# svip-lab/impersonator

Hardware: NVIDIA H100
Metric: frames/sec @256x256 (per-frame inference hot path) (higher is better)
Workload: dtype f16 main product + e4m3 correction products (hi/lo split), f32 accumulate

## Files before the change

impersonator_b200/csrc/conv_tc.cu:

```cuda
#include <cuda.h>

#include <stdlib.h>

#include <algorithm>
#include <new>
#include <type_traits>

#include "common.cuh"

namespace {

constexpr int TILE_H = 16, TILE_W = 8;
constexpr int SWAP_N_TILE = 64;
constexpr int SWAP_TILE_H = 32;
constexpr int KCHUNK = 64;
constexpr int ROW_BYTES = TILE_W * 128;
constexpr int MAX_TAPS = 49;
constexpr int MAX_GROUP = 8;
constexpr int RING_BYTES = 200 * 1024;
constexpr int MAX_STAGES = 8;
constexpr int NUM_CONSUMERS = 256;
constexpr int NUM_THREADS = NUM_CONSUMERS + 128;
constexpr int MAX_N_TILE = 128;
static_assert(2 * 2 * (TILE_H + MAX_GROUP - 1) * ROW_BYTES + 2 * 2 * MAX_N_TILE * 128 <= RING_BYTES,
              "every plan needs two A and two B entries in the ring");
static_assert(2 * 2 * (SWAP_TILE_H + MAX_GROUP - 1) * ROW_BYTES + 2 * 2 * SWAP_N_TILE * 128 <= RING_BYTES,
              "every swapped plan needs two A and two B entries in the ring");
static_assert(SWAP_N_TILE * (SWAP_TILE_H * TILE_W) == MAX_N_TILE * (TILE_H * TILE_W), "same accumulator budget");

__host__ __device__ constexpr int tile_rows(int n_tile) { return n_tile == SWAP_N_TILE ? SWAP_TILE_H : TILE_H; }

struct ConvParams {
    CUtensorMap a_hi[4];
    CUtensorMap a_lo[4];
    CUtensorMap w_hi;
    CUtensorMap w_lo;
    int n_img, tiles_y, tiles_x, n_tiles_n;
    int dom_h, dom_w;
    int ntaps, chunks0, chunks1;
    signed char dy[MAX_TAPS], dx[MAX_TAPS], tmap[MAX_TAPS];
    short wtap[MAX_TAPS];
    int ngroups;
    signed char g_first[MAX_TAPS], g_cnt[MAX_TAPS];
    int a_rows;
    int a_stages, b_stages;
    float* out; int out_h, out_w, cout;
    int oy_mul, oy_add, ox_mul, ox_add;
    double* stats;
    float out_scale;
    int phase_cols;
};

template <int N_TILE, bool SPLIT>
struct Cfg {
    static constexpr int B_BYTES = N_TILE * 128;
    static constexpr int B_STAGE_BYTES = B_BYTES * (SPLIT ? 2 : 1);
    static constexpr int BAR_BYTES = 4 * MAX_STAGES * 8;
    static constexpr int STATS_PARTS = N_TILE < SWAP_N_TILE ? 8 : N_TILE == SWAP_N_TILE ? 2 : 0;
    static constexpr int STATS_BYTES = STATS_PARTS * N_TILE * 8;
    static constexpr int SMEM_BYTES = 1024 + RING_BYTES + BAR_BYTES + STATS_BYTES;
    static_assert(B_STAGE_BYTES % 1024 == 0, "B entries must keep the 1024-byte swizzle alignment");
    static_assert(SMEM_BYTES <= 227 * 1024, "exceeds the shared memory of a block");
};

__device__ __forceinline__ uint32_t smem_u32(const void* p) { return (uint32_t)__cvta_generic_to_shared(p); }

__device__ __forceinline__ void mbar_init(uint64_t* bar, uint32_t count) {
    asm volatile("mbarrier.init.shared::cta.b64 [%0], %1;" ::"r"(smem_u32(bar)), "r"(count));
}
__device__ __forceinline__ void mbar_expect_tx(uint64_t* bar, uint32_t bytes) {
    asm volatile("mbarrier.arrive.expect_tx.shared::cta.b64 _, [%0], %1;" ::"r"(smem_u32(bar)), "r"(bytes) : "memory");
}
__device__ __forceinline__ void mbar_arrive(uint64_t* bar) {
    asm volatile("mbarrier.arrive.shared::cta.b64 _, [%0];" ::"r"(smem_u32(bar)) : "memory");
}
__device__ __forceinline__ bool mbar_try_wait(uint64_t* bar, uint32_t parity) {
    uint32_t ok;
    asm volatile("{\n\t.reg .pred p;\n\t"
                 "mbarrier.try_wait.parity.shared::cta.b64 p, [%1], %2;\n\t"
                 "selp.u32 %0, 1, 0, p;\n\t}"
                 : "=r"(ok) : "r"(smem_u32(bar)), "r"(parity) : "memory");
    return ok != 0;
}
__device__ __forceinline__ void mbar_wait(uint64_t* bar, uint32_t parity) {
    if (mbar_try_wait(bar, parity)) return;
    const long long t0 = clock64();
    while (!mbar_try_wait(bar, parity)) {
        if (clock64() - t0 > 4000000000ll) __trap();
    }
}
__device__ __forceinline__ bool elect_one() {
    uint32_t pred;
    asm volatile("{\n\t.reg .pred P;\n\telect.sync _|P, 0xffffffff;\n\tselp.b32 %0, 1, 0, P;\n\t}" : "=r"(pred));
    return pred != 0;
}
__device__ __forceinline__ void fence_barrier_init() { asm volatile("fence.mbarrier_init.release.cluster;" ::: "memory"); }
__device__ __forceinline__ void fence_proxy_async() { asm volatile("fence.proxy.async.shared::cta;" ::: "memory"); }

__device__ __forceinline__ void tma_load_4d(const CUtensorMap* map, void* dst, uint64_t* bar, int c0, int c1, int c2, int c3) {
    asm volatile("cp.async.bulk.tensor.4d.shared::cluster.global.mbarrier::complete_tx::bytes [%0], [%1, {%3, %4, %5, %6}], [%2];"
                 :: "r"(smem_u32(dst)), "l"(map), "r"(smem_u32(bar)), "r"(c0), "r"(c1), "r"(c2), "r"(c3) : "memory");
}
__device__ __forceinline__ void tma_load_3d(const CUtensorMap* map, void* dst, uint64_t* bar, int c0, int c1, int c2) {
    asm volatile("cp.async.bulk.tensor.3d.shared::cluster.global.mbarrier::complete_tx::bytes [%0], [%1, {%3, %4, %5}], [%2];"
                 :: "r"(smem_u32(dst)), "l"(map), "r"(smem_u32(bar)), "r"(c0), "r"(c1), "r"(c2) : "memory");
}

__device__ __forceinline__ uint64_t make_desc(uint32_t smem_addr) {
    return (uint64_t)((smem_addr & 0x3FFFF) >> 4) | (1ull << 16) | (64ull << 32) | (1ull << 62);
}
__device__ __forceinline__ void wgmma_fence() { asm volatile("wgmma.fence.sync.aligned;" ::: "memory"); }
__device__ __forceinline__ void wgmma_commit() { asm volatile("wgmma.commit_group.sync.aligned;" ::: "memory"); }
template <int N>
__device__ __forceinline__ void wgmma_wait() { asm volatile("wgmma.wait_group.sync.aligned %0;" :: "n"(N) : "memory"); }
__device__ __forceinline__ void acc_fence(float& r) { asm volatile("" : "+f"(r) :: "memory"); }

template <int N> __device__ __forceinline__ void wgmma_f16(float* d, uint64_t da, uint64_t db);
template <int N> __device__ __forceinline__ void wgmma_e4m3(float* d, uint64_t da, uint64_t db);
template <> __device__ __forceinline__ void wgmma_f16<16>(float* d, uint64_t da, uint64_t db) {
    asm volatile("{\n\t.reg .pred p;\n\tsetp.ne.b32 p, %10, 0;\n\t"
                 "wgmma.mma_async.sync.aligned.m64n16k16.f32.f16.f16 {%0, %1, %2, %3, %4, %5, %6, %7}, %8, %9, p, 1, 1, 0, 0;\n\t}"
                 : "+f"(d[0]), "+f"(d[1]), "+f"(d[2]), "+f"(d[3]), "+f"(d[4]), "+f"(d[5]), "+f"(d[6]), "+f"(d[7])
                 : "l"(da), "l"(db), "r"(1));
}
template <> __device__ __forceinline__ void wgmma_f16<32>(float* d, uint64_t da, uint64_t db) {
    asm volatile("{\n\t.reg .pred p;\n\tsetp.ne.b32 p, %18, 0;\n\t"
                 "wgmma.mma_async.sync.aligned.m64n32k16.f32.f16.f16 {%0, %1, %2, %3, %4, %5, %6, %7, %8, %9, %10, %11, %12, %13, %14, %15}, %16, %17, p, 1, 1, 0, 0;\n\t}"
                 : "+f"(d[0]), "+f"(d[1]), "+f"(d[2]), "+f"(d[3]), "+f"(d[4]), "+f"(d[5]), "+f"(d[6]), "+f"(d[7]), "+f"(d[8]), "+f"(d[9]), "+f"(d[10]), "+f"(d[11]), "+f"(d[12]), "+f"(d[13]), "+f"(d[14]), "+f"(d[15])
                 : "l"(da), "l"(db), "r"(1));
}
template <> __device__ __forceinline__ void wgmma_f16<128>(float* d, uint64_t da, uint64_t db) {
    asm volatile("{\n\t.reg .pred p;\n\tsetp.ne.b32 p, %66, 0;\n\t"
                 "wgmma.mma_async.sync.aligned.m64n128k16.f32.f16.f16 {%0, %1, %2, %3, %4, %5, %6, %7, %8, %9, %10, %11, %12, %13, %14, %15, %16, %17, %18, %19, %20, %21, %22, %23, %24, %25, %26, %27, %28, %29, %30, %31, %32, %33, %34, %35, %36, %37, %38, %39, %40, %41, %42, %43, %44, %45, %46, %47, %48, %49, %50, %51, %52, %53, %54, %55, %56, %57, %58, %59, %60, %61, %62, %63}, %64, %65, p, 1, 1, 0, 0;\n\t}"
                 : "+f"(d[0]), "+f"(d[1]), "+f"(d[2]), "+f"(d[3]), "+f"(d[4]), "+f"(d[5]), "+f"(d[6]), "+f"(d[7]), "+f"(d[8]), "+f"(d[9]), "+f"(d[10]), "+f"(d[11]), "+f"(d[12]), "+f"(d[13]), "+f"(d[14]), "+f"(d[15]), "+f"(d[16]), "+f"(d[17]), "+f"(d[18]), "+f"(d[19]), "+f"(d[20]), "+f"(d[21]), "+f"(d[22]), "+f"(d[23]), "+f"(d[24]), "+f"(d[25]), "+f"(d[26]), "+f"(d[27]), "+f"(d[28]), "+f"(d[29]), "+f"(d[30]), "+f"(d[31]), "+f"(d[32]), "+f"(d[33]), "+f"(d[34]), "+f"(d[35]), "+f"(d[36]), "+f"(d[37]), "+f"(d[38]), "+f"(d[39]), "+f"(d[40]), "+f"(d[41]), "+f"(d[42]), "+f"(d[43]), "+f"(d[44]), "+f"(d[45]), "+f"(d[46]), "+f"(d[47]), "+f"(d[48]), "+f"(d[49]), "+f"(d[50]), "+f"(d[51]), "+f"(d[52]), "+f"(d[53]), "+f"(d[54]), "+f"(d[55]), "+f"(d[56]), "+f"(d[57]), "+f"(d[58]), "+f"(d[59]), "+f"(d[60]), "+f"(d[61]), "+f"(d[62]), "+f"(d[63])
                 : "l"(da), "l"(db), "r"(1));
}
template <> __device__ __forceinline__ void wgmma_e4m3<16>(float* d, uint64_t da, uint64_t db) {
    asm volatile("{\n\t.reg .pred p;\n\tsetp.ne.b32 p, %10, 0;\n\t"
                 "wgmma.mma_async.sync.aligned.m64n16k32.f32.e4m3.e4m3 {%0, %1, %2, %3, %4, %5, %6, %7}, %8, %9, p, 1, 1;\n\t}"
                 : "+f"(d[0]), "+f"(d[1]), "+f"(d[2]), "+f"(d[3]), "+f"(d[4]), "+f"(d[5]), "+f"(d[6]), "+f"(d[7])
                 : "l"(da), "l"(db), "r"(1));
}
template <> __device__ __forceinline__ void wgmma_e4m3<32>(float* d, uint64_t da, uint64_t db) {
    asm volatile("{\n\t.reg .pred p;\n\tsetp.ne.b32 p, %18, 0;\n\t"
                 "wgmma.mma_async.sync.aligned.m64n32k32.f32.e4m3.e4m3 {%0, %1, %2, %3, %4, %5, %6, %7, %8, %9, %10, %11, %12, %13, %14, %15}, %16, %17, p, 1, 1;\n\t}"
                 : "+f"(d[0]), "+f"(d[1]), "+f"(d[2]), "+f"(d[3]), "+f"(d[4]), "+f"(d[5]), "+f"(d[6]), "+f"(d[7]), "+f"(d[8]), "+f"(d[9]), "+f"(d[10]), "+f"(d[11]), "+f"(d[12]), "+f"(d[13]), "+f"(d[14]), "+f"(d[15])
                 : "l"(da), "l"(db), "r"(1));
}
template <> __device__ __forceinline__ void wgmma_e4m3<128>(float* d, uint64_t da, uint64_t db) {
    asm volatile("{\n\t.reg .pred p;\n\tsetp.ne.b32 p, %66, 0;\n\t"
                 "wgmma.mma_async.sync.aligned.m64n128k32.f32.e4m3.e4m3 {%0, %1, %2, %3, %4, %5, %6, %7, %8, %9, %10, %11, %12, %13, %14, %15, %16, %17, %18, %19, %20, %21, %22, %23, %24, %25, %26, %27, %28, %29, %30, %31, %32, %33, %34, %35, %36, %37, %38, %39, %40, %41, %42, %43, %44, %45, %46, %47, %48, %49, %50, %51, %52, %53, %54, %55, %56, %57, %58, %59, %60, %61, %62, %63}, %64, %65, p, 1, 1;\n\t}"
                 : "+f"(d[0]), "+f"(d[1]), "+f"(d[2]), "+f"(d[3]), "+f"(d[4]), "+f"(d[5]), "+f"(d[6]), "+f"(d[7]), "+f"(d[8]), "+f"(d[9]), "+f"(d[10]), "+f"(d[11]), "+f"(d[12]), "+f"(d[13]), "+f"(d[14]), "+f"(d[15]), "+f"(d[16]), "+f"(d[17]), "+f"(d[18]), "+f"(d[19]), "+f"(d[20]), "+f"(d[21]), "+f"(d[22]), "+f"(d[23]), "+f"(d[24]), "+f"(d[25]), "+f"(d[26]), "+f"(d[27]), "+f"(d[28]), "+f"(d[29]), "+f"(d[30]), "+f"(d[31]), "+f"(d[32]), "+f"(d[33]), "+f"(d[34]), "+f"(d[35]), "+f"(d[36]), "+f"(d[37]), "+f"(d[38]), "+f"(d[39]), "+f"(d[40]), "+f"(d[41]), "+f"(d[42]), "+f"(d[43]), "+f"(d[44]), "+f"(d[45]), "+f"(d[46]), "+f"(d[47]), "+f"(d[48]), "+f"(d[49]), "+f"(d[50]), "+f"(d[51]), "+f"(d[52]), "+f"(d[53]), "+f"(d[54]), "+f"(d[55]), "+f"(d[56]), "+f"(d[57]), "+f"(d[58]), "+f"(d[59]), "+f"(d[60]), "+f"(d[61]), "+f"(d[62]), "+f"(d[63])
                 : "l"(da), "l"(db), "r"(1));
}

__device__ __forceinline__ void consumer_sync() { asm volatile("bar.sync 1, 256;" ::: "memory"); }

struct TileCoord {
    int n_idx, img, y0, x0;
};
template <int TH>
__device__ __forceinline__ TileCoord decode_tile(const ConvParams& P, int tile, int m_tiles) {
    TileCoord t;
    t.n_idx = tile / m_tiles;
    const int m_idx = tile % m_tiles;
    t.img = m_idx / (P.tiles_y * P.tiles_x);
    const int rem = m_idx % (P.tiles_y * P.tiles_x);
    t.y0 = (rem / P.tiles_x) * TH; t.x0 = (rem % P.tiles_x) * TILE_W;
    return t;
}

template <int N_TILE>
__device__ __forceinline__ void warp_tile_stats(const float* acc, bool v0, bool v1, int warp, unsigned lane, float2* s_stats)
{
#pragma unroll
    for (int j = 0; j < N_TILE / 8; j++) {
        const float a0 = v0 ? acc[4 * j] : 0.f, a1 = v0 ? acc[4 * j + 1] : 0.f;
        const float b0 = v1 ? acc[4 * j + 2] : 0.f, b1 = v1 ? acc[4 * j + 3] : 0.f;
        float s0 = a0 + b0, s1 = a1 + b1, q0 = a0 * a0 + b0 * b0, q1 = a1 * a1 + b1 * b1;
#pragma unroll
        for (int off = 4; off <= 16; off <<= 1) {
            s0 += __shfl_xor_sync(0xffffffffu, s0, off); s1 += __shfl_xor_sync(0xffffffffu, s1, off);
            q0 += __shfl_xor_sync(0xffffffffu, q0, off); q1 += __shfl_xor_sync(0xffffffffu, q1, off);
        }
        if (lane < 4) {
            s_stats[warp * N_TILE + 8 * j + 2 * lane] = make_float2(s0, q0);
            s_stats[warp * N_TILE + 8 * j + 2 * lane + 1] = make_float2(s1, q1);
        }
    }
}

template <int N_TILE, int PARTS>
__device__ __forceinline__ void flush_tile_stats(const ConvParams& P, const float2* s_stats, int img, int n_idx)
{
    consumer_sync();
    for (int col = threadIdx.x; col < N_TILE; col += NUM_CONSUMERS) {
        float s = 0.f, q = 0.f;
#pragma unroll
        for (int w = 0; w < PARTS; w++) { const float2 v = s_stats[w * N_TILE + col]; s += v.x; q += v.y; }
        int ch = n_idx * N_TILE + col;
        if (P.phase_cols > 0) ch %= P.phase_cols;
        double* dst = P.stats + 2 * ((size_t)img * P.cout + ch);
        atomicAdd(dst, (double)s);
        atomicAdd(dst + 1, (double)q);
    }
    consumer_sync();
}

template <int N_TILE>
__device__ __forceinline__ void epilogue_plain(const ConvParams& P, float* acc, const TileCoord& t, int warp, unsigned lane,
                                               float2* s_stats)
{
    const int tx = (int)(lane >> 2), x = t.x0 + tx;
    const int y[2] = {t.y0 + 2 * warp, t.y0 + 2 * warp + 1};
    const bool valid[2] = {y[0] < P.dom_h && x < P.dom_w, y[1] < P.dom_h && x < P.dom_w};
    if (P.out_scale != 1.f) {
#pragma unroll
        for (int i = 0; i < N_TILE / 2; i++) acc[i] *= P.out_scale;
    }
    if (P.out) {
        const int out_w_c = P.out_w * P.cout;
#pragma unroll
        for (int h = 0; h < 2; h++) {
            if (!valid[h]) continue;
            float* optr = P.out + (((size_t)t.img * P.out_h + (P.oy_mul * y[h] + P.oy_add)) * P.out_w + (P.ox_mul * x + P.ox_add)) * P.cout
                        + (size_t)t.n_idx * N_TILE;
#pragma unroll
            for (int j = 0; j < N_TILE / 8; j++) {
                const int c = 8 * j + 2 * (int)(lane & 3);
                float* o = optr + c;
                if (P.phase_cols > 0) {
                    const int col = t.n_idx * N_TILE + c, ph = col / P.phase_cols;
                    o = P.out + (((size_t)t.img * P.out_h + 2 * y[h]) * P.out_w + 2 * x) * P.cout
                      + (size_t)(ph >> 1) * out_w_c + (ph & 1) * P.cout + (col - ph * P.phase_cols);
                }
                *reinterpret_cast<float2*>(o) = make_float2(acc[4 * j + 2 * h], acc[4 * j + 2 * h + 1]);
            }
        }
    }
    if (P.stats) {
        warp_tile_stats<N_TILE>(acc, valid[0], valid[1], warp, lane, s_stats);
        flush_tile_stats<N_TILE, 8>(P, s_stats, t.img, t.n_idx);
    }
}

template <int N_TILE>
__device__ __forceinline__ void epilogue_channel_major(const ConvParams& P, float* acc, const TileCoord& t, int warp,
                                                       unsigned lane, float2* s_stats)
{
    const int wg = warp >> 2;
    const int c_base = N_TILE == MAX_N_TILE ? 64 * wg : 0, row0 = N_TILE == MAX_N_TILE ? 0 : 16 * wg;
    const int c0 = c_base + 16 * (warp & 3) + (int)(lane >> 2);
    const int y0 = t.y0 + row0, x0 = t.x0 + 2 * (int)(lane & 3);
    const int rows = P.dom_h - y0;
    const bool vx[2] = {x0 < P.dom_w, x0 + 1 < P.dom_w};
    const int col = t.n_idx * N_TILE + c0;
    const int ph = P.phase_cols > 0 ? col / P.phase_cols : 0;
    const int ch = col - ph * P.phase_cols;
    const size_t coff = ((size_t)(ph >> 1) * P.out_w + (ph & 1)) * P.cout + ch;
    if (P.out_scale != 1.f) {
#pragma unroll
        for (int i = 0; i < 64; i++) acc[i] *= P.out_scale;
    }
    if (P.out) {
#pragma unroll
        for (int j = 0; j < 16; j++) {
            if (j >= rows) break;
            const size_t orow = ((size_t)t.img * P.out_h + (P.oy_mul * (y0 + j) + P.oy_add)) * P.out_w;
#pragma unroll
            for (int e = 0; e < 2; e++) {
                if (!vx[e]) continue;
                float* o = P.out + (orow + (P.ox_mul * (x0 + e) + P.ox_add)) * P.cout;
                o[coff] = acc[4 * j + e];
                o[coff + 8] = acc[4 * j + 2 + e];
            }
        }
    }
    if (P.stats) {
        float s[2] = {0.f, 0.f}, q[2] = {0.f, 0.f};
#pragma unroll
        for (int j = 0; j < 16; j++) {
#pragma unroll
            for (int e = 0; e < 2; e++) {
                const bool v = j < rows && vx[e];
#pragma unroll
                for (int h = 0; h < 2; h++) {
                    const float a = v ? acc[4 * j + 2 * h + e] : 0.f;
                    s[h] += a; q[h] += a * a;
                }
            }
        }
#pragma unroll
        for (int h = 0; h < 2; h++) {
#pragma unroll
            for (int off = 1; off <= 2; off <<= 1) {
                s[h] += __shfl_xor_sync(0xffffffffu, s[h], off);
                q[h] += __shfl_xor_sync(0xffffffffu, q[h], off);
            }
        }
        if constexpr (N_TILE == SWAP_N_TILE) {
            if ((lane & 3) == 0) {
                s_stats[wg * N_TILE + c0] = make_float2(s[0], q[0]);
                s_stats[wg * N_TILE + c0 + 8] = make_float2(s[1], q[1]);
            }
            flush_tile_stats<N_TILE, 2>(P, s_stats, t.img, t.n_idx);
        } else if ((lane & 3) == 0) {
#pragma unroll
            for (int h = 0; h < 2; h++) {
                double* dst = P.stats + 2 * ((size_t)t.img * P.cout + ch + 8 * h);
                atomicAdd(dst, (double)s[h]);
                atomicAdd(dst + 1, (double)q[h]);
            }
        }
    }
}

enum { MODE_FP16 = 0, MODE_FP16X3 = 1, MODE_F8 = 2 };

template <int N_TILE, int MODE>
struct Regs {
    static constexpr int CONSUMER = N_TILE >= 64 ? (MODE == MODE_F8 ? 168 : 120) : N_TILE == 32 ? 80 : 64;
    static constexpr int LAUNCH = ((2 * CONSUMER + 40 + 2) / 3 + 7) / 8 * 8;
    static constexpr int PRODUCER = 3 * LAUNCH - 2 * CONSUMER;
    static_assert(PRODUCER >= 40 && PRODUCER % 8 == 0 && CONSUMER % 8 == 0, "setmaxnreg takes multiples of 8");
};

template <int N_TILE, bool CM>
__device__ __forceinline__ void mma_f16(float* d, uint64_t act, uint64_t w) {
    if constexpr (CM) wgmma_f16<128>(d, w, act);
    else              wgmma_f16<N_TILE>(d, act, w);
}
template <int N_TILE, bool CM>
__device__ __forceinline__ void mma_e4m3(float* d, uint64_t act, uint64_t w) {
    if constexpr (CM) wgmma_e4m3<128>(d, w, act);
    else              wgmma_e4m3<N_TILE>(d, act, w);
}

template <int N_TILE, int MODE>
__global__ void __launch_bounds__(NUM_THREADS, 1) __maxnreg__((Regs<N_TILE, MODE>::LAUNCH))
k_conv_wg(const __grid_constant__ ConvParams P)
{
    constexpr bool CM = N_TILE >= SWAP_N_TILE;
    constexpr bool SPLIT = MODE != MODE_FP16;
    constexpr int TH = N_TILE == SWAP_N_TILE ? SWAP_TILE_H : TILE_H;
    constexpr int ACC = CM ? 64 : N_TILE / 2;
    using C = Cfg<N_TILE, SPLIT>;
    extern __shared__ uint8_t smem_raw[];
    uint8_t* smem = reinterpret_cast<uint8_t*>((reinterpret_cast<uintptr_t>(smem_raw) + 1023) & ~(uintptr_t)1023);
    const int a_op_bytes = P.a_rows * ROW_BYTES;
    const int a_stage_bytes = a_op_bytes * (SPLIT ? 2 : 1);
    uint8_t* b_ring = smem + P.a_stages * a_stage_bytes;
    uint64_t* a_full = reinterpret_cast<uint64_t*>(smem + RING_BYTES);
    uint64_t* a_empty = a_full + MAX_STAGES;
    uint64_t* b_full = a_empty + MAX_STAGES;
    uint64_t* b_empty = b_full + MAX_STAGES;
    float2* s_stats = reinterpret_cast<float2*>(smem + RING_BYTES + C::BAR_BYTES);

    const int warp = threadIdx.x >> 5;
    const unsigned lane = threadIdx.x & 31;

    if (threadIdx.x == 0) {
        for (int s = 0; s < P.a_stages; s++) { mbar_init(a_full + s, 1); mbar_init(a_empty + s, NUM_CONSUMERS / 32); }
        for (int s = 0; s < P.b_stages; s++) { mbar_init(b_full + s, 1); mbar_init(b_empty + s, NUM_CONSUMERS / 32); }
        fence_barrier_init();
        fence_proxy_async();
    }
    __syncthreads();
    lwb::pdl_wait();
    lwb::pdl_trigger();

    const int nchunks = P.chunks0 + P.chunks1;
    const int m_tiles = P.n_img * P.tiles_y * P.tiles_x;
    const int total = m_tiles * P.n_tiles_n;

    if (warp >= NUM_CONSUMERS / 32) {
        asm volatile("setmaxnreg.dec.sync.aligned.u32 %0;" :: "n"(Regs<N_TILE, MODE>::PRODUCER));
        if (warp != NUM_CONSUMERS / 32) return;
        if (elect_one()) {
            asm volatile("prefetch.tensormap [%0];" :: "l"(&P.a_hi[0]) : "memory");
            asm volatile("prefetch.tensormap [%0];" :: "l"(&P.w_hi) : "memory");
            if (SPLIT) {
                asm volatile("prefetch.tensormap [%0];" :: "l"(&P.a_lo[0]) : "memory");
                asm volatile("prefetch.tensormap [%0];" :: "l"(&P.w_lo) : "memory");
            }
        }
        int as = 0, bs = 0; uint32_t aph = 0, bph = 0;
        for (int tile = blockIdx.x; tile < total; tile += gridDim.x) {
            const TileCoord t = decode_tile<TH>(P, tile, m_tiles);
            for (int g = 0; g < P.ngroups; g++) {
                const int first = P.g_first[g], cnt = P.g_cnt[g];
                const int xx = t.x0 + P.dx[first], yy = t.y0 + P.dy[first];
                for (int chunk = 0; chunk < nchunks; chunk++) {
                    const bool second = chunk >= P.chunks0;
                    const int mi = second ? 1 : P.tmap[first];
                    const int c0 = (second ? chunk - P.chunks0 : chunk) * KCHUNK;
                    mbar_wait(a_empty + as, aph ^ 1);
                    uint8_t* sa = smem + as * a_stage_bytes;
                    if (elect_one()) {
                        mbar_expect_tx(a_full + as, (uint32_t)a_stage_bytes);
                        tma_load_4d(&P.a_hi[mi], sa, a_full + as, c0, xx, yy, t.img);
                        if (SPLIT) tma_load_4d(&P.a_lo[mi], sa + a_op_bytes, a_full + as, c0, xx, yy, t.img);
                    }
                    __syncwarp();
                    if (++as == P.a_stages) { as = 0; aph ^= 1; }
                    for (int i = 0; i < cnt; i++) {
                        mbar_wait(b_empty + bs, bph ^ 1);
                        uint8_t* sb = b_ring + bs * C::B_STAGE_BYTES;
                        const int wt = P.wtap[first + i];
                        if (elect_one()) {
                            mbar_expect_tx(b_full + bs, (uint32_t)C::B_STAGE_BYTES);
                            tma_load_3d(&P.w_hi, sb, b_full + bs, chunk * KCHUNK, t.n_idx * N_TILE, wt);
                            if (SPLIT) tma_load_3d(&P.w_lo, sb + C::B_BYTES, b_full + bs, chunk * KCHUNK, t.n_idx * N_TILE, wt);
                        }
                        __syncwarp();
                        if (++bs == P.b_stages) { bs = 0; bph ^= 1; }
                    }
                }
            }
        }
    } else {
        asm volatile("setmaxnreg.inc.sync.aligned.u32 %0;" :: "n"(Regs<N_TILE, MODE>::CONSUMER));
        constexpr bool CH_SPLIT = N_TILE == MAX_N_TILE;
        const uint32_t wg = (uint32_t)(warp >> 2);
        const uint32_t a_base = smem_u32(smem) + (CH_SPLIT ? 0 : wg * (TH / 2) * ROW_BYTES);
        const uint32_t b_base = smem_u32(b_ring) + (CH_SPLIT ? wg * 64 * 128 : 0);
        float acc[ACC];
        float acc8[MODE == MODE_F8 ? ACC : 1];
        int as = 0, bs = 0; uint32_t aph = 0, bph = 0;
        for (int tile = blockIdx.x; tile < total; tile += gridDim.x) {
            const TileCoord t = decode_tile<TH>(P, tile, m_tiles);
#pragma unroll
            for (int i = 0; i < ACC; i++) acc[i] = 0.f;
#pragma unroll
            for (int i = 0; i < (MODE == MODE_F8 ? ACC : 1); i++) acc8[i] = 0.f;
            int prev_b = -1, prev_a = -1;
            for (int g = 0; g < P.ngroups; g++) {
                const int cnt = P.g_cnt[g];
                for (int chunk = 0; chunk < nchunks; chunk++) {
                    mbar_wait(a_full + as, aph);
                    const uint32_t a_hi = a_base + as * a_stage_bytes;
                    for (int i = 0; i < cnt; i++) {
                        mbar_wait(b_full + bs, bph);
                        const uint32_t ai = a_hi + i * ROW_BYTES, al = ai + a_op_bytes;
                        const uint32_t b_hi = b_base + bs * C::B_STAGE_BYTES, b_lo = b_hi + C::B_BYTES;
                        wgmma_fence();
#pragma unroll
                        for (int k = 0; k < KCHUNK / 16; k++) {
                            const uint64_t da = make_desc(ai + k * 32), db = make_desc(b_hi + k * 32);
                            mma_f16<N_TILE, CM>(acc, da, db);
                            if constexpr (MODE == MODE_F8) {
                                mma_e4m3<N_TILE, CM>(acc8, make_desc(al + k * 32), make_desc(b_lo + k * 32));
                            } else if constexpr (MODE == MODE_FP16X3) {
                                mma_f16<N_TILE, CM>(acc, da, make_desc(b_lo + k * 32));
                                mma_f16<N_TILE, CM>(acc, make_desc(al + k * 32), db);
                            }
                        }
                        wgmma_commit();
                        if (prev_b >= 0) {
                            wgmma_wait<1>();
                            if (lane == 0) {
                                mbar_arrive(b_empty + prev_b);
                                if (prev_a >= 0) mbar_arrive(a_empty + prev_a);
                            }
                            prev_a = -1;
                        }
                        prev_b = bs;
                        if (++bs == P.b_stages) { bs = 0; bph ^= 1; }
                    }
                    prev_a = as;
                    if (++as == P.a_stages) { as = 0; aph ^= 1; }
                }
            }
            wgmma_wait<0>();
#pragma unroll
            for (int i = 0; i < ACC; i++) acc_fence(acc[i]);
            if constexpr (MODE == MODE_F8) {
#pragma unroll
                for (int i = 0; i < ACC; i++) { acc_fence(acc8[i]); acc[i] += acc8[i]; }
            }
            if (lane == 0) { mbar_arrive(b_empty + prev_b); mbar_arrive(a_empty + prev_a); }
            if constexpr (CM) epilogue_channel_major<N_TILE>(P, acc, t, warp, lane, s_stats);
            else              epilogue_plain<N_TILE>(P, acc, t, warp, lane, s_stats);
        }
    }
}

typedef CUresult (*EncodeTiledFn)(CUtensorMap*, CUtensorMapDataType, cuuint32_t, void*, const cuuint64_t*,
                                  const cuuint64_t*, const cuuint32_t*, const cuuint32_t*, CUtensorMapInterleave,
                                  CUtensorMapSwizzle, CUtensorMapL2promotion, CUtensorMapFloatOOBfill);

EncodeTiledFn get_encode()
{
    static EncodeTiledFn fn = nullptr;
    if (!fn) {
        void* p = nullptr;
        cudaDriverEntryPointQueryResult q;
        if (cudaGetDriverEntryPoint("cuTensorMapEncodeTiled", &p, cudaEnableDefault, &q) != cudaSuccess || !p) return nullptr;
        fn = (EncodeTiledFn)p;
    }
    return fn;
}

int encode_map(CUtensorMap* m, const void* base, int rank, const uint64_t* dims, const uint64_t* strides_bytes, const uint32_t* box)
{
    EncodeTiledFn enc = get_encode();
    if (!enc) { lwb::set_error("cuTensorMapEncodeTiled entry point not available"); return LWB_E_CUDA; }
    cuuint64_t gdim[5]; cuuint64_t gstr[4]; cuuint32_t bx[5]; cuuint32_t es[5];
    for (int i = 0; i < rank; i++) { gdim[i] = dims[i]; bx[i] = box[i]; es[i] = 1; }
    for (int i = 0; i < rank - 1; i++) gstr[i] = strides_bytes[i];
    CUresult r = enc(m, CU_TENSOR_MAP_DATA_TYPE_FLOAT16, (cuuint32_t)rank, const_cast<void*>(base), gdim, gstr, bx, es,
                     CU_TENSOR_MAP_INTERLEAVE_NONE, CU_TENSOR_MAP_SWIZZLE_128B, CU_TENSOR_MAP_L2_PROMOTION_L2_256B,
                     CU_TENSOR_MAP_FLOAT_OOB_FILL_NONE);
    if (r != CUDA_SUCCESS) {
        lwb::set_error("cuTensorMapEncodeTiled failed (%d): rank %d dims [%llu,%llu,%llu,%llu] strides [%llu,%llu,%llu] box [%u,%u,%u,%u]",
                       (int)r, rank, (unsigned long long)dims[0], (unsigned long long)dims[1], (unsigned long long)(rank > 2 ? dims[2] : 0),
                       (unsigned long long)(rank > 3 ? dims[3] : 0), (unsigned long long)strides_bytes[0],
                       (unsigned long long)(rank > 2 ? strides_bytes[1] : 0), (unsigned long long)(rank > 3 ? strides_bytes[2] : 0),
                       box[0], box[1], rank > 2 ? box[2] : 0, rank > 3 ? box[3] : 0);
        return LWB_E_CUDA;
    }
    return LWB_OK;
}

struct Launch {
    ConvParams p;
    int n_tile;
    int mode;
    int grid;
};

template <int N_TILE, int MODE>
int launch_wg(const Launch& L, cudaStream_t st)
{
    using C = Cfg<N_TILE, MODE != MODE_FP16>;
    static bool attr_set_dev[lwb::kMaxDevices] = {};
    bool& attr_set = attr_set_dev[lwb::device_slot()];
    if (!attr_set) {
        LWB_CUDA_OK(cudaFuncSetAttribute(k_conv_wg<N_TILE, MODE>, cudaFuncAttributeMaxDynamicSharedMemorySize, C::SMEM_BYTES));
        attr_set = true;
    }
    LWB_CUDA_OK(lwb::launch_pdl(k_conv_wg<N_TILE, MODE>, dim3(L.grid), dim3(NUM_THREADS), C::SMEM_BYTES, st, L.p));
    LWB_LAUNCH_OK();
    return LWB_OK;
}

template <class F>
int with_instance(int n_tile, int mode, F&& f)
{
    auto modes = [&](auto nt) {
        if (mode == MODE_F8) return f(nt, std::integral_constant<int, MODE_F8>());
        if (mode == MODE_FP16X3) return f(nt, std::integral_constant<int, MODE_FP16X3>());
        return f(nt, std::integral_constant<int, MODE_FP16>());
    };
    switch (n_tile) {
        case 16:  return modes(std::integral_constant<int, 16>());
        case 32:  return modes(std::integral_constant<int, 32>());
        case 64:  return modes(std::integral_constant<int, 64>());
        case 128: return modes(std::integral_constant<int, 128>());
    }
    lwb::set_error("conv_tc: unsupported N tile %d", n_tile);
    return LWB_E_UNSUPPORTED;
}

int launch(const Launch& L, cudaStream_t st)
{
    return with_instance(L.n_tile, L.mode,
                         [&](auto nt, auto md) { return launch_wg<decltype(nt)::value, decltype(md)::value>(L, st); });
}

int pick_n_tile(int cout, int forced)
{
    if (forced > 0) return forced > MAX_N_TILE && forced % MAX_N_TILE == 0 ? MAX_N_TILE : forced;
    if (cout % 128 == 0) return 128;
    if (cout % 64 == 0) return 64;
    if (cout % 32 == 0) return 32;
    if (cout % 16 == 0) return 16;
    return -1;
}

struct View {
    const uint16_t* hi;
    const uint16_t* lo;
    uint64_t dims[4], str[3];
};

struct LaunchSpec {
    int ntaps;
    signed char dy[MAX_TAPS], dx[MAX_TAPS], tmap[MAX_TAPS];
    short wtap[MAX_TAPS];
    int chunks0, chunks1;
    int nviews;
    View a[4];
    View w;
    int ncols;
    int dom_h, dom_w;
    int oy_mul, oy_add, ox_mul, ox_add, phase_cols;
    int n_tile;

    void tap(int y, int x, int view, int wt)
    {
        dy[ntaps] = (signed char)y; dx[ntaps] = (signed char)x; tmap[ntaps] = (signed char)view; wtap[ntaps] = (short)wt;
        ntaps++;
    }
};

}

struct lwb_conv_plan {
    int num;
    Launch launches[4];
};

static View nhwc_view(const uint16_t* hi, const uint16_t* lo, int n, int h, int w, int c, int step = 1, int py = 0, int px = 0)
{
    const size_t off = ((size_t)py * w + px) * c;
    return View{hi + off, lo ? lo + off : lo,
                {(uint64_t)c, (uint64_t)((w - px + step - 1) / step), (uint64_t)((h - py + step - 1) / step), (uint64_t)n},
                {(uint64_t)step * c * 2, (uint64_t)step * w * c * 2, (uint64_t)h * w * c * 2}};
}

static View weight_view(const uint16_t* hi, const uint16_t* lo, int k, int ncols, int taps)
{
    return View{hi, lo, {(uint64_t)k, (uint64_t)ncols, (uint64_t)taps}, {(uint64_t)k * 2, (uint64_t)ncols * k * 2}};
}

static int encode_pair(CUtensorMap* hi, CUtensorMap* lo, int rank, const View& v, const uint32_t* box, bool split)
{
    const int rc = encode_map(hi, v.hi, rank, v.dims, v.str, box);
    return rc != LWB_OK || !split ? rc : encode_map(lo, v.lo, rank, v.dims, v.str, box);
}

static void group_taps(ConvParams& p, int tile_h)
{
    int order[MAX_TAPS];
    for (int t = 0; t < p.ntaps; t++) order[t] = t;
    std::stable_sort(order, order + p.ntaps, [&](int a, int b) {
        if (p.tmap[a] != p.tmap[b]) return p.tmap[a] < p.tmap[b];
        if (p.dx[a] != p.dx[b]) return p.dx[a] < p.dx[b];
        return p.dy[a] < p.dy[b];
    });
    const ConvParams src = p;
    int longest = 0;
    p.ngroups = 0;
    for (int t = 0; t < p.ntaps; t++) {
        const int o = order[t];
        p.dy[t] = src.dy[o]; p.dx[t] = src.dx[o]; p.tmap[t] = src.tmap[o]; p.wtap[t] = src.wtap[o];
        const bool joins = t > 0 && p.tmap[t] == p.tmap[t - 1] && p.dx[t] == p.dx[t - 1] && p.dy[t] == p.dy[t - 1] + 1 &&
                           p.g_cnt[p.ngroups - 1] < MAX_GROUP;
        if (!joins) { p.g_first[p.ngroups] = (signed char)t; p.g_cnt[p.ngroups] = 0; p.ngroups++; }
        p.g_cnt[p.ngroups - 1]++;
        longest = std::max(longest, (int)p.g_cnt[p.ngroups - 1]);
    }
    p.a_rows = tile_h + longest - 1;
}

static void pick_rings(ConvParams& p, int n_tile, bool split)
{
    const int ops = split ? 2 : 1;
    const int a_bytes = p.a_rows * ROW_BYTES * ops, b_bytes = n_tile * 128 * ops;
    const int longest = p.a_rows - tile_rows(n_tile) + 1;
    int best = 0;
    for (int a = 2; a <= MAX_STAGES; a++) {
        const int b = std::min(MAX_STAGES, (RING_BYTES - a * a_bytes) / b_bytes);
        if (b < 2) break;
        if (std::min(a * longest, b) > best) { best = std::min(a * longest, b); p.a_stages = a; p.b_stages = b; }
    }
}

static int build_launch(Launch& L, const LaunchSpec& s, const lwb_conv_desc* d, float* out_raw, double* stats, int sms)
{
    const bool split = d->split != 0;
    ConvParams& p = L.p;
    memset(&p, 0, sizeof(p));
    p.ntaps = s.ntaps; p.chunks0 = s.chunks0; p.chunks1 = s.chunks1;
    for (int t = 0; t < s.ntaps; t++) { p.dy[t] = s.dy[t]; p.dx[t] = s.dx[t]; p.tmap[t] = s.tmap[t]; p.wtap[t] = s.wtap[t]; }
    group_taps(p, tile_rows(s.n_tile));
    int rc;
    const uint32_t a_box[4] = {KCHUNK, TILE_W, (uint32_t)p.a_rows, 1};
    for (int v = 0; v < s.nviews; v++)
        if ((rc = encode_pair(&p.a_hi[v], &p.a_lo[v], 4, s.a[v], a_box, split)) != LWB_OK) return rc;
    const uint32_t w_box[3] = {KCHUNK, (uint32_t)s.n_tile, 1};
    if ((rc = encode_pair(&p.w_hi, &p.w_lo, 3, s.w, w_box, split)) != LWB_OK) return rc;
    p.n_img = d->n;
    p.dom_h = s.dom_h; p.dom_w = s.dom_w;
    p.tiles_y = lwb::ceil_div(s.dom_h, tile_rows(s.n_tile)); p.tiles_x = lwb::ceil_div(s.dom_w, TILE_W);
    p.n_tiles_n = s.ncols / s.n_tile;
    p.out = out_raw; p.out_h = d->h_out; p.out_w = d->w_out; p.cout = d->cout;
    p.oy_mul = s.oy_mul; p.oy_add = s.oy_add; p.ox_mul = s.ox_mul; p.ox_add = s.ox_add; p.phase_cols = s.phase_cols;
    p.stats = stats;
    p.out_scale = ldexpf(1.f, -d->w_exp);
    L.n_tile = s.n_tile; L.mode = d->split;
    pick_rings(p, s.n_tile, split);
    const long total = (long)p.n_img * p.tiles_y * p.tiles_x * p.n_tiles_n;
    L.grid = (int)(total < sms ? total : sms);
    return LWB_OK;
}

extern "C" int lwb_conv_plan_create(const lwb_conv_desc* d,
                                    const uint16_t* x0_hi, const uint16_t* x0_lo,
                                    const uint16_t* x1_hi, const uint16_t* x1_lo,
                                    const uint16_t* w_hi, const uint16_t* w_lo,
                                    float* out_raw, double* stats, lwb_conv_plan** plan_out)
{
    LWB_CHECK_ARG(d && x0_hi && w_hi && out_raw && plan_out, "null pointer");
    const bool split = d->split != 0;
    const bool f8 = d->split == 2;
    LWB_CHECK_ARG(d->split >= 0 && d->split <= 2, "split must be 0, 1 or 2");
    LWB_CHECK_ARG(!split || (x0_lo && w_lo), "split mode needs the lo operands");
    LWB_CHECK_ARG(!f8 || (!d->rowk && !d->halo), "the fp8 lo mode is not available for row-K / halo plans");
    LWB_CHECK_ARG(d->n > 0 && d->h_in > 0 && d->w_in > 0 && d->cout > 0, "non-positive size");
    LWB_CHECK_ARG(d->cout % 16 == 0, "cout must be a multiple of 16");
    LWB_CHECK_ARG(d->w_exp >= -40 && d->w_exp <= 60, "w_exp out of range");
    const int n_tile = pick_n_tile(d->cout, d->n_tile);
    LWB_CHECK_ARG(n_tile > 0 && d->cout % n_tile == 0, "no N tile divides cout");
    if (d->halo) {
        LWB_CHECK_ARG(d->stride == 1 && !d->transposed && d->dil == 1, "halo mode needs stride 1, dilation 1, not transposed");
        if (d->rowk) LWB_CHECK_ARG(d->kw <= 8 && d->cin0 == 8 && d->cin1 == 0 && d->row_pitch >= d->w_in + 8, "row-K shape");
        else         LWB_CHECK_ARG(d->kw <= 9 && (d->kw & 1) && (d->kh & 1), "halo mode needs an odd kernel, kw <= 9, with 'same' padding (kh/2, kw/2)");
    }

    const int sms = lwb::sm_count();

    LaunchSpec s = {};
    s.n_tile = n_tile; s.ncols = d->cout;
    s.dom_h = d->h_out; s.dom_w = d->w_out;
    s.oy_mul = s.ox_mul = 1;
    s.nviews = 1;
    LaunchSpec specs[4];
    int num = 1;
    if (d->rowk) {
        LWB_CHECK_ARG(d->stride == 1 && !d->transposed && d->kw <= 8 && d->cin0 == 8 && d->cin1 == 0, "row-K needs stride 1, kw <= 8, 8 channels");
        LWB_CHECK_ARG(d->h_out == d->h_in && d->w_out == d->w_in && d->row_pitch >= d->w_in + 8, "row-K shape");
        for (int ky = 0; ky < d->kh; ky++) s.tap(ky, 0, 0, ky);
        s.chunks0 = 1;
        const uint64_t hp = d->h_in + d->kh - 1, row_bytes = (uint64_t)d->row_pitch * 16;
        s.a[0] = View{x0_hi, x0_lo, {64, (uint64_t)d->w_in, hp, (uint64_t)d->n}, {16, row_bytes, hp * row_bytes}};
        s.w = weight_view(w_hi, w_lo, 64, d->cout, d->kh);
    } else {
        LWB_CHECK_ARG(d->cin0 % KCHUNK == 0 && d->cin1 % KCHUNK == 0 && d->cin0 > 0, "input channels must be multiples of 64");
        LWB_CHECK_ARG(d->cin1 == 0 || (x1_hi && (!split || x1_lo)), "second input missing");
        const int cin_total = d->cin0 + d->cin1;
        const int ntaps_w = d->kh * d->kw;
        LWB_CHECK_ARG(ntaps_w <= MAX_TAPS, "too many filter taps");
        s.chunks0 = d->cin0 / KCHUNK; s.chunks1 = d->cin1 / KCHUNK;
        s.a[0] = nhwc_view(x0_hi, x0_lo, d->n, d->h_in, d->w_in, d->cin0);
        s.w = weight_view(w_hi, w_lo, cin_total, d->cout, ntaps_w);
        if (d->transposed) {
            LWB_CHECK_ARG(d->kh == 3 && d->kw == 3 && d->stride == 2 && d->pad == 1 && d->cin1 == 0, "transposed conv: only k3 s2 p1 op1");
            LWB_CHECK_ARG(d->h_out == 2 * d->h_in && d->w_out == 2 * d->w_in, "transposed conv output must be 2x input");
            s.dom_h = d->h_in; s.dom_w = d->w_in;
            s.oy_mul = s.ox_mul = 2;
        }
        if (d->transposed == 2) {
            s.n_tile = MAX_N_TILE;
            s.ncols = 4 * d->cout;
            LWB_CHECK_ARG(d->cout % 32 == 0 && s.ncols % s.n_tile == 0, "merged transposed conv needs cout in multiples of 32");
            for (int t = 0; t < 4; t++) s.tap(t >> 1, t & 1, 0, t);
            s.w = weight_view(w_hi, w_lo, cin_total, s.ncols, 4);
            s.phase_cols = d->cout;
        } else if (d->transposed) {
            const int ky_list[2][2] = {{1, -1}, {2, 0}}, d_list[2][2] = {{0, 0}, {0, 1}}, cnt[2] = {1, 2};
            num = 4;
            for (int a = 0; a < 2; a++) for (int b = 0; b < 2; b++) {
                LaunchSpec& q = specs[a * 2 + b];
                q = s;
                for (int i = 0; i < cnt[a]; i++) for (int j = 0; j < cnt[b]; j++)
                    q.tap(d_list[a][i], d_list[b][j], 0, ky_list[a][i] * 3 + ky_list[b][j]);
                q.oy_add = a; q.ox_add = b;
            }
        } else {
            LWB_CHECK_ARG(d->stride == 1 || d->stride == 2, "stride must be 1 or 2");
            LWB_CHECK_ARG(d->stride == 1 || d->cin1 == 0, "concat input only with stride 1");
            const int st = d->stride;
            for (int ky = 0; ky < d->kh; ky++) for (int kx = 0; kx < d->kw; kx++) {
                const int oy = ky * d->dil - d->pad, ox = kx * d->dil - (d->pad_w >= 0 ? d->pad_w : d->pad);
                if (oy < -127 || oy > 127 || ox < -127 || ox > 127) { lwb::set_error("conv_tc: tap offset out of range"); return LWB_E_UNSUPPORTED; }
                const int py = ((oy % st) + st) % st, px = ((ox % st) + st) % st;
                s.tap((oy - py) / st, (ox - px) / st, py * 2 + px, s.ntaps);
            }
            s.nviews = st * st;
            for (int v = 0; v < s.nviews; v++) s.a[v] = nhwc_view(x0_hi, x0_lo, d->n, d->h_in, d->w_in, d->cin0, st, v >> 1, v & 1);
            if (d->cin1) {
                s.nviews = 2;
                s.a[1] = nhwc_view(x1_hi, x1_lo, d->n, d->h_in, d->w_in, d->cin1);
            }
        }
    }
    if (num == 1) specs[0] = s;

    lwb_conv_plan* plan = new (std::nothrow) lwb_conv_plan();
    LWB_CHECK_ARG(plan, "out of host memory");
    for (; plan->num < num; plan->num++) {
        const int rc = build_launch(plan->launches[plan->num], specs[plan->num], d, out_raw, stats, sms);
        if (rc != LWB_OK) { delete plan; return rc; }
    }
    *plan_out = plan;
    return LWB_OK;
}

extern "C" int lwb_conv_plan_run(const lwb_conv_plan* plan, lwb_stream_t stream)
{
    LWB_CHECK_ARG(plan, "null plan");
    for (int i = 0; i < plan->num; i++) {
        const int rc = launch(plan->launches[i], (cudaStream_t)stream);
        if (rc != LWB_OK) return rc;
    }
    return LWB_OK;
}

extern "C" void lwb_conv_plan_destroy(lwb_conv_plan* plan) { delete plan; }

extern "C" int lwb_conv_plan_num_launches(const lwb_conv_plan* plan) { return plan ? plan->num : 0; }

extern "C" int lwb_conv2d_nhwc(const lwb_conv_desc* d,
                               const uint16_t* x0_hi, const uint16_t* x0_lo,
                               const uint16_t* x1_hi, const uint16_t* x1_lo,
                               const uint16_t* w_hi, const uint16_t* w_lo,
                               float* out_raw, double* stats, lwb_stream_t stream)
{
    lwb_conv_plan* plan = nullptr;
    int rc = lwb_conv_plan_create(d, x0_hi, x0_lo, x1_hi, x1_lo, w_hi, w_lo, out_raw, stats, &plan);
    if (rc != LWB_OK) return rc;
    rc = lwb_conv_plan_run(plan, stream);
    lwb_conv_plan_destroy(plan);
    return rc;
}

template <int N_TILE, int MODE>
static int conv_resources(int* out)
{
    using C = Cfg<N_TILE, MODE != MODE_FP16>;
    cudaFuncAttributes a;
    LWB_CUDA_OK(cudaFuncSetAttribute(k_conv_wg<N_TILE, MODE>, cudaFuncAttributeMaxDynamicSharedMemorySize, C::SMEM_BYTES));
    LWB_CUDA_OK(cudaFuncGetAttributes(&a, k_conv_wg<N_TILE, MODE>));
    int blocks = 0;
    LWB_CUDA_OK(cudaOccupancyMaxActiveBlocksPerMultiprocessor(&blocks, k_conv_wg<N_TILE, MODE>, NUM_THREADS, C::SMEM_BYTES));
    out[0] = a.numRegs; out[1] = (int)a.sharedSizeBytes; out[2] = C::SMEM_BYTES; out[3] = (int)a.localSizeBytes;
    out[4] = NUM_THREADS; out[5] = blocks; out[6] = Regs<N_TILE, MODE>::CONSUMER;
    return LWB_OK;
}

extern "C" int lwb_conv_kernel_resources(int n_tile, int mode, int* out)
{
    LWB_CHECK_ARG(out, "null pointer");
    LWB_CHECK_ARG(mode >= 0 && mode <= 2, "mode must be 0, 1 or 2");
    return with_instance(n_tile, mode,
                         [&](auto nt, auto md) { return conv_resources<decltype(nt)::value, decltype(md)::value>(out); });
}
```

Baseline: 2269.

## Assign contiguous tile ranges and carry channel stats in shared memory across tiles

For the channel-major path, each block now takes a contiguous range of tiles instead of a grid-strided set. Per-channel sum and sum-of-squares are accumulated in double precision in shared-memory carry slots across consecutive tiles of the same image. They are flushed with global atomics only at an image boundary or at the end of the range. This removes the per-tile consumer barrier and the per-tile double atomics on the stats buffer, but contiguous assignment may worsen load balance and L2 locality compared with striding.

```diff
diff --git a/impersonator_b200/csrc/conv_tc.cu b/impersonator_b200/csrc/conv_tc.cu
--- a/impersonator_b200/csrc/conv_tc.cu
+++ b/impersonator_b200/csrc/conv_tc.cu
@@ -56,8 +56,8 @@
     static constexpr int B_BYTES = N_TILE * 128;
     static constexpr int B_STAGE_BYTES = B_BYTES * (SPLIT ? 2 : 1);
     static constexpr int BAR_BYTES = 4 * MAX_STAGES * 8;
-    static constexpr int STATS_PARTS = N_TILE < SWAP_N_TILE ? 8 : N_TILE == SWAP_N_TILE ? 2 : 0;
-    static constexpr int STATS_BYTES = STATS_PARTS * N_TILE * 8;
+    static constexpr int CARRY_SLOTS = 2 * (NUM_CONSUMERS / 4);
+    static constexpr int STATS_BYTES = N_TILE < SWAP_N_TILE ? 8 * N_TILE * 8 : CARRY_SLOTS * 16;
     static constexpr int SMEM_BYTES = 1024 + RING_BYTES + BAR_BYTES + STATS_BYTES;
     static_assert(B_STAGE_BYTES % 1024 == 0, "B entries must keep the 1024-byte swizzle alignment");
     static_assert(SMEM_BYTES <= 227 * 1024, "exceeds the shared memory of a block");
@@ -156,6 +156,20 @@
 
 __device__ __forceinline__ void consumer_sync() { asm volatile("bar.sync 1, 256;" ::: "memory"); }
 
+struct TileRange {
+    int first, end, step;
+};
+template <bool CM>
+__device__ __forceinline__ TileRange tile_range(int total)
+{
+    if constexpr (CM) {
+        const int b = (int)blockIdx.x, q = total / (int)gridDim.x, r = total % (int)gridDim.x;
+        const int first = b * q + min(b, r);
+        return {first, first + q + (b < r ? 1 : 0), 1};
+    } else {
+        return {(int)blockIdx.x, total, (int)gridDim.x};
+    }
+}
 struct TileCoord {
     int n_idx, img, y0, x0;
 };
@@ -190,14 +204,14 @@
     }
 }
 
-template <int N_TILE, int PARTS>
+template <int N_TILE>
 __device__ __forceinline__ void flush_tile_stats(const ConvParams& P, const float2* s_stats, int img, int n_idx)
 {
     consumer_sync();
     for (int col = threadIdx.x; col < N_TILE; col += NUM_CONSUMERS) {
         float s = 0.f, q = 0.f;
 #pragma unroll
-        for (int w = 0; w < PARTS; w++) { const float2 v = s_stats[w * N_TILE + col]; s += v.x; q += v.y; }
+        for (int w = 0; w < NUM_CONSUMERS / 32; w++) { const float2 v = s_stats[w * N_TILE + col]; s += v.x; q += v.y; }
         int ch = n_idx * N_TILE + col;
         if (P.phase_cols > 0) ch %= P.phase_cols;
         double* dst = P.stats + 2 * ((size_t)img * P.cout + ch);
@@ -240,13 +254,13 @@
     }
     if (P.stats) {
         warp_tile_stats<N_TILE>(acc, valid[0], valid[1], warp, lane, s_stats);
-        flush_tile_stats<N_TILE, 8>(P, s_stats, t.img, t.n_idx);
+        flush_tile_stats<N_TILE>(P, s_stats, t.img, t.n_idx);
     }
 }
 
 template <int N_TILE>
 __device__ __forceinline__ void epilogue_channel_major(const ConvParams& P, float* acc, const TileCoord& t, int warp,
-                                                       unsigned lane, float2* s_stats)
+                                                       unsigned lane, double2* carry, bool flush)
 {
     const int wg = warp >> 2;
     const int c_base = N_TILE == MAX_N_TILE ? 64 * wg : 0, row0 = N_TILE == MAX_N_TILE ? 0 : 16 * wg;
@@ -298,18 +312,19 @@
                 q[h] += __shfl_xor_sync(0xffffffffu, q[h], off);
             }
         }
-        if constexpr (N_TILE == SWAP_N_TILE) {
-            if ((lane & 3) == 0) {
-                s_stats[wg * N_TILE + c0] = make_float2(s[0], q[0]);
-                s_stats[wg * N_TILE + c0 + 8] = make_float2(s[1], q[1]);
-            }
-            flush_tile_stats<N_TILE, 2>(P, s_stats, t.img, t.n_idx);
-        } else if ((lane & 3) == 0) {
+        if ((lane & 3) == 0) {
+            double2* slot = carry + 16 * warp + (lane >> 2);
 #pragma unroll
             for (int h = 0; h < 2; h++) {
-                double* dst = P.stats + 2 * ((size_t)t.img * P.cout + ch + 8 * h);
-                atomicAdd(dst, (double)s[h]);
-                atomicAdd(dst + 1, (double)q[h]);
+                double2 v = slot[8 * h];
+                v.x += (double)s[h]; v.y += (double)q[h];
+                if (flush) {
+                    double* dst = P.stats + 2 * ((size_t)t.img * P.cout + ch + 8 * h);
+                    atomicAdd(dst, v.x);
+                    atomicAdd(dst + 1, v.y);
+                    v = make_double2(0.0, 0.0);
+                }
+                slot[8 * h] = v;
             }
         }
     }
@@ -355,10 +370,12 @@
     uint64_t* b_full = a_empty + MAX_STAGES;
     uint64_t* b_empty = b_full + MAX_STAGES;
     float2* s_stats = reinterpret_cast<float2*>(smem + RING_BYTES + C::BAR_BYTES);
+    double2* carry = reinterpret_cast<double2*>(s_stats);
 
     const int warp = threadIdx.x >> 5;
     const unsigned lane = threadIdx.x & 31;
 
+    if (CM && threadIdx.x < C::CARRY_SLOTS) carry[threadIdx.x] = make_double2(0.0, 0.0);
     if (threadIdx.x == 0) {
         for (int s = 0; s < P.a_stages; s++) { mbar_init(a_full + s, 1); mbar_init(a_empty + s, NUM_CONSUMERS / 32); }
         for (int s = 0; s < P.b_stages; s++) { mbar_init(b_full + s, 1); mbar_init(b_empty + s, NUM_CONSUMERS / 32); }
@@ -372,6 +389,7 @@
     const int nchunks = P.chunks0 + P.chunks1;
     const int m_tiles = P.n_img * P.tiles_y * P.tiles_x;
     const int total = m_tiles * P.n_tiles_n;
+    const TileRange run = tile_range<CM>(total);
 
     if (warp >= NUM_CONSUMERS / 32) {
         asm volatile("setmaxnreg.dec.sync.aligned.u32 %0;" :: "n"(Regs<N_TILE, MODE>::PRODUCER));
@@ -385,7 +403,7 @@
             }
         }
         int as = 0, bs = 0; uint32_t aph = 0, bph = 0;
-        for (int tile = blockIdx.x; tile < total; tile += gridDim.x) {
+        for (int tile = run.first; tile < run.end; tile += run.step) {
             const TileCoord t = decode_tile<TH>(P, tile, m_tiles);
             for (int g = 0; g < P.ngroups; g++) {
                 const int first = P.g_first[g], cnt = P.g_cnt[g];
@@ -426,8 +444,9 @@
         const uint32_t b_base = smem_u32(b_ring) + (CH_SPLIT ? wg * 64 * 128 : 0);
         float acc[ACC];
         float acc8[MODE == MODE_F8 ? ACC : 1];
+        const int img_tiles = P.tiles_y * P.tiles_x;
         int as = 0, bs = 0; uint32_t aph = 0, bph = 0;
-        for (int tile = blockIdx.x; tile < total; tile += gridDim.x) {
+        for (int tile = run.first; tile < run.end; tile += run.step) {
             const TileCoord t = decode_tile<TH>(P, tile, m_tiles);
 #pragma unroll
             for (int i = 0; i < ACC; i++) acc[i] = 0.f;
@@ -479,8 +498,12 @@
                 for (int i = 0; i < ACC; i++) { acc_fence(acc8[i]); acc[i] += acc8[i]; }
             }
             if (lane == 0) { mbar_arrive(b_empty + prev_b); mbar_arrive(a_empty + prev_a); }
-            if constexpr (CM) epilogue_channel_major<N_TILE>(P, acc, t, warp, lane, s_stats);
-            else              epilogue_plain<N_TILE>(P, acc, t, warp, lane, s_stats);
+            if constexpr (CM) {
+                const bool flush = tile + 1 == run.end || (tile + 1) % img_tiles == 0;
+                epilogue_channel_major<N_TILE>(P, acc, t, warp, lane, carry, flush);
+            } else {
+                epilogue_plain<N_TILE>(P, acc, t, warp, lane, s_stats);
+            }
         }
     }
 }
```

After: 2306 (median of 6 runs). Within noise of the previous version (+1.6%).
